# Jiraiya812/Fast-CU-Decision-HEVC

Measured on AMD Instinct MI355X. Metric: CTUs/sec (RDO decision only) at 4K all-intra, higher is better.
Workload: dtype int32+f64

## Files before the change

### fast-cu-decision-hevc_amd/csrc/fcu_engine.h

```cpp
#pragma once
#include <stdint.h>
#include <string.h>
#include <type_traits>
#include "../../include/fcu.h"

#ifdef FCU_EMU
#include <math.h>
#include <stdio.h>
#include <stdlib.h>
#define FCU_DEV static inline
#define FCU_MEMBER inline
#define FCU_NOINLINE
#define FCU_INLINE
#define FCU_TABLE static const
static int g_emu_phase = 0, g_emu_in_phase = 0, g_emu_lane = 0, g_emu_relax = 0;
#define FCU_EMU_RELAX(on) (g_emu_relax = (on))
static inline int fcu_emu_phase_begin() { g_emu_phase++; g_emu_in_phase = 1; g_emu_lane = 0; return 0; }
static inline int fcu_emu_phase_next(int lane) { if (lane + 1 >= 64) g_emu_in_phase = 0; g_emu_lane = lane + 1; return lane + 1; }
template <class T> static inline T fcu_emu_uni(T v, int site, int line)
{
  enum { SITES = 2048, K = 32, B = 16 };
  struct Seen { int phase, first, cur, idx, n; unsigned char vals[K][B]; };
  static Seen seen[SITES];
  if (g_emu_in_phase && !g_emu_relax && sizeof(T) <= B && site < SITES) {
// ... 5 lines not shown
    s.idx++;
  }
  return v;
}
#define FCU_FOR_LANES for (int lane = fcu_emu_phase_begin(); lane < 64; lane = fcu_emu_phase_next(lane))
#define FCU_ATOMIC_ADD(p, v) (*(p) += (v))
#define FCU_ATOMIC_MAX(p, v) do { if (*(p) < (v)) *(p) = (v); } while (0)
#define FCU_ATOMIC_OR(p, v) (*(p) |= (v))
#define FCU_WAVE_ADD(p, v) (*(p) += (v))
#define FCU_WAVE_MIN64(p, v) do { if ((v) < *(p)) *(p) = (v); } while (0)
#define FCU_IN_LDS(p) do { } while (0)
#define FCU_UNI(x) fcu_emu_uni((x), __COUNTER__, __LINE__)
#define FCU_HBM
#define FCU_FLOOR(x) floor(x)
#define FCU_CHECK(c) do { if (!(c)) { fprintf(stderr, "FCU_CHECK failed: %s (line %d)\n", #c, __LINE__); abort(); } } while (0)
#else
#define FCU_DEV __device__ static
#define FCU_MEMBER __device__ inline
#define FCU_NOINLINE __noinline__
#define FCU_INLINE __attribute__((always_inline))
#define FCU_TABLE __device__ static const
#define FCU_FOR_LANES for (int lane = (int)threadIdx.x, fcu_once_ = 1; fcu_once_; fcu_once_ = 0, __syncthreads())
#define FCU_ATOMIC_ADD(p, v) atomicAdd((p), (v))
#define FCU_ATOMIC_MAX(p, v) atomicMax((p), (v))
#define FCU_ATOMIC_OR(p, v) atomicOr((p), (v))
__device__ inline uint32_t fcu_wave_sum(uint32_t v)
{
  v += (uint32_t)__builtin_amdgcn_update_dpp(0, (int)v, 0xb1, 0xf, 0xf, false);
  v += (uint32_t)__builtin_amdgcn_update_dpp(0, (int)v, 0x4e, 0xf, 0xf, false);
  v += (uint32_t)__builtin_amdgcn_update_dpp(0, (int)v, 0x124, 0xf, 0xf, false);
// ... 44 lines not shown
#define FCU_QTIC(v) long long v = clock64()
#define FCU_QTOC(E_, v, idx) do { if (threadIdx.x == 0) (E_).C->prof[idx] += (unsigned long long)(clock64() - v); v = clock64(); } while (0)
#define FCU_TOC(E_, v, idx) do { if ((idx) == 10 && threadIdx.x == 0) (E_).C->prof[idx] += (unsigned long long)(clock64() - v); } while (0)
#define FCU_COUNT(E_, idx, n) do { } while (0)
#elif defined(FCU_PROFILE_INTER)
#define FCU_ITOC(E_, v, idx) do { if (threadIdx.x == 0) (E_).C->prof[idx] += (unsigned long long)(clock64() - v); } while (0)
#define FCU_TOC(E_, v, idx) do { if ((idx) == 10 && threadIdx.x == 0) (E_).C->prof[idx] += (unsigned long long)(clock64() - v); } while (0)
#define FCU_COUNT(E_, idx, n) do { } while (0)
#elif defined(FCU_PROFILE_RDOQ) || defined(FCU_PROFILE_DEPTH)
#define FCU_TOC(E_, v, idx) do { if ((idx) < 11 && threadIdx.x == 0) (E_).C->prof[idx] += (unsigned long long)(clock64() - v); } while (0)
#define FCU_COUNT(E_, idx, n) do { } while (0)
#elif defined(FCU_PROFILE_RMD)
#define FCU_MTOC(E_, v, idx) do { if (threadIdx.x == 0) (E_).C->prof[idx] += (unsigned long long)(clock64() - v); } while (0)
#define FCU_TOC(E_, v, idx) do { if ((idx) < 11 && threadIdx.x == 0) (E_).C->prof[idx] += (unsigned long long)(clock64() - v); } while (0)
#define FCU_COUNT(E_, idx, n) do { } while (0)
#else
#define FCU_TOC(E_, v, idx) do { if (threadIdx.x == 0) (E_).C->prof[idx] += (unsigned long long)(clock64() - v); } while (0)
#define FCU_COUNT(E_, idx, n) do { (E_).C->prof[idx] += (unsigned long long)(n); } while (0)
#endif
#else
#define FCU_TIC(v) do { } while (0)
#define FCU_TOC(E_, v, idx) do { } while (0)
#define FCU_COUNT(E_, idx, n) do { } while (0)
#endif
#ifndef FCU_QTOC
#define FCU_QTIC(v) do { } while (0)
#define FCU_QTOC(E_, v, idx) do { } while (0)
#endif
#ifndef FCU_ITOC
#define FCU_ITOC(E_, v, idx) do { } while (0)
#endif
#ifndef FCU_MTOC
#define FCU_MTOC(E_, v, idx) do { } while (0)
#endif

#include "fcu_tables.h"

struct HotTables { uint32_t bin[256]; uint16_t scan[3][16]; uint8_t scan_cg8[3][4]; uint8_t ctx_ind_map4x4[16]; uint8_t group_idx[32];
                   uint64_t scan4_nib[3], map4_nib; uint32_t cnt_bits[4]; };
#ifdef FCU_EMU
static HotTables g_hot;
#else
__shared__ HotTables g_hot;
#endif

#if defined(FCU_PROFILE_RQT) && !defined(FCU_EMU)
#define FCU_RTIC(v) long long v = clock64()
#define FCU_RTOC(P_, v, idx) do { if (!SER && threadIdx.x == 0) { ((Chain *)((char *)&(P_) - __builtin_offsetof(Chain, p)))->prof[idx] += (unsigned long long)(clock64() - v); v = clock64(); } } while (0)
// ... 101 lines not shown
  Yuv16 resi_cu, resi_best, qt_resi[4];
  Yuv tmp_pred;
  uint8_t me_pred[9][CTU * CTU];
  int16_t me_h[3][72 * 64];
  int par_ps[4];
  int memo_valid[4][MEMO_K], memo_next[4], memo_zero[4][MEMO_K];
  int16_t memo_mv[4][MEMO_K][NPART][2]; int8_t memo_ref[4][MEMO_K][NPART];
  uint8_t memo_tr_idx[4][MEMO_K][NPART], memo_cbf[4][MEMO_K][3][NPART], memo_tskip[4][MEMO_K][3][NPART];
  alignas(16) int16_t memo_coef[MEMO_K * MEMO_POOL], memo_resi[MEMO_K * MEMO_POOL];
};

struct Env { Chain *C; Scratch *G; int cur_ctu, slice_start; };
struct TU { int log2, tr_depth, part, nparts, x, y, off_y, cw, cwo, cx, cy, c_tr_depth, c_code_all, off_c, cu_depth, plast; };

struct Shared {
  Cabac cab[1 + (MAXDEPTH + 1) + MAXLC];
  uint8_t ref5[5][68]; int dc5[5]; uint32_t cm_dist[5];
  union {
    int16_t lane_abs[MAXLC][32];
    RdoqRec rq_rec[16];
    struct {
      int32_t colsum[128];
      union {
        struct { uint8_t ref[264], reff[264]; };
        uint8_t ref5b[5][68];
      };
    };
  };
  union {
    int16_t rq_lv[16];
    uint32_t sad[36];
// ... 21 lines not shown
      uint32_t tz_best; int tz_bx, tz_by, tz_dist, tz_round, tz_point;
      int mrg_buf[5], best_is_skip, me_out[4];
    };
  };
  int pu_best_vc, pu_best_mode, pu_nvc; uint32_t pu_best_dist; double pu_best_cost;
  int t_abs, t_lsp, t_last; uint32_t t_dist;
  int rw_abs, rw_lsp;
  double q_cost[4]; uint32_t q_dist[4];
  int c_best_mode; uint32_t c_best_dist; double c_best_cost; int c_modes[5];
  uint32_t c_dist;
  Env env;
  TU wk_st[4]; int wk_ci[4]; int wk_part[4], wk_child[4];
  double cand_cost[12];
  uint32_t c64_dist[5]; uint8_t c64_cbf[5][4]; int c64_valid;
  uint64_t q_frac[5], t_frac;
  double dec_j0, dec_j1; int dec_cnt, dec_flip;
};

enum { CAB_GOON = 0, CAB_CUR0 = 1, CAB_LANE0 = 1 + (MAXDEPTH + 1) };
enum { EST_CODERS = 7 };
static_assert(EST_CODERS * sizeof(Cabac) >= NCTX_INTRA * 2 * sizeof(uint32_t) && EST_CODERS <= MAXLC, "est table does not fit its lane coders");
#define FCU_EST ((uint32_t *)&g_S.cab[CAB_LANE0 + MAXLC - EST_CODERS])
enum { RMD_STAGE_BYTES = 64 * 8 * 2, RMD_COST_BYTES = 35 * 8 };
static_assert(RMD_STAGE_BYTES + RMD_COST_BYTES <= MAXLC * sizeof(Cabac) && (CAB_LANE0 * sizeof(Cabac)) % 8 == 0, "RMD staging does not fit the lane coders");
#define FCU_RMD_STAGE ((int16_t *)&g_S.cab[CAB_LANE0])
#define FCU_RMD_COST ((double *)((char *)&g_S.cab[CAB_LANE0] + RMD_STAGE_BYTES))
FCU_DEV int ref_key(int px, int py, int log2) { return px | (py << 13) | (log2 << 26); }
#ifdef FCU_EMU
static Shared g_S;
#else
__shared__ Shared g_S;
#endif
FCU_DEV Env env_get() { return FCU_UNI(g_S.env); }
FCU_DEV Cabac *slot_ptr(const Env E, int d, int ci) { return ci == CI_CURR_BEST ? &g_S.cab[CAB_CUR0 + d] : &E.G->slots[d][ci]; }
// ... 1279 lines not shown
  const Env E = env_get(); c = FCU_UNI(c); cu = FCU_UNI(cu); const TU tu = tu_of_key(FCU_UNI(tu_k));
  const int part = tu.part, partSize = cu->part_size[0], log2 = tu.log2;
  cab_reset_bits(c);
  if (part == 0 && E.C->p.slice_type != SLICE_I) { code_skip_flag(E, c, cu, 0); code_pred_mode(c, cu, 0); }
  if (part == 0 && cu->depth[0] == MAXDEPTH) cab_bin(c, partSize == SIZE_2Nx2N, CTX_PARTSIZE);
  if (partSize == SIZE_2Nx2N ? (part == 0) : (tu.tr_depth > 0 && (part & ((cu->nparts >> 2) - 1)) == 0))
    code_luma_dir_bits(c, cu->intra_dir[0][part], g_S.preds);
  if (!(partSize == SIZE_NxN && tu.tr_depth == 0) && log2 != LOG2_MINTU && log2 != min_tu_log2_in_cu(cu->depth[part], cu->part_size[part]))
    cab_bin(c, 0, CTX_SUBDIV + 5 - log2);
  const int cbf = g_S.t_abs > 0;
  cab_bin(c, cbf, CTX_CBF_LUMA + (tu.tr_depth == 0 ? 1 : 0));
  if (cbf) code_coeff_body<1>(c, E.G->p_qscan, 1, g_S.t_lsp, log2, 0, coef_scan_idx(cu->intra_dir[0][part], log2, 0), cu->tskip[0][part], E.C->p, g_S.lane_abs[0]);
  return cab_bits(c);
}

FCU_DEV FCU_NOINLINE void encode_transform(int c, const CuObj *cu, int cuPart, uint32_t root_k)
{
  const Env E = env_get(); c = FCU_UNI(c); cu = FCU_UNI(cu); cuPart = FCU_UNI(cuPart); const TU root = tu_of_key(FCU_UNI(root_k));
  TU *st = g_S.wk_st; int *ci = g_S.wk_ci; int sp = 0;
  st[0] = root; ci[0] = -1;
  while (sp >= 0) {
    const TU tu = st[sp];
    if (ci[sp] < 0) {
      const int part = cuPart + tu.part, trIdx = tu.tr_depth, subdiv = cu->tr_idx[part] > trIdx;
      if (cu->part_size[part] == SIZE_NxN && trIdx == 0) { }
      else if (tu.log2 > LOG2_MAXTU) { }
      else if (tu.log2 == LOG2_MINTU) { }
      else if (tu.log2 == min_tu_log2_in_cu(cu->depth[part], cu->part_size[part])) { }
      else cab_bin(c, subdiv, CTX_SUBDIV + 5 - tu.log2);
      const int first = trIdx == 0;
      for (int comp = 1; comp < 3; comp++)
        if (first || tu.c_code_all)
          if (first || ((cu->cbf[comp][part] >> (trIdx - 1)) & 1)) {
            const int lowest = trIdx + ((subdiv && !(tu.cwo >= 8)) ? 1 : 0);
            cab_bin(c, (cu->cbf[comp][cuPart + tu_part_c(tu)] >> lowest) & 1, CTX_CBF_CHROMA + trIdx);
          }
      if (!subdiv) {
        cab_bin(c, (cu->cbf[0][part] >> trIdx) & 1, CTX_CBF_LUMA + (trIdx == 0 ? 1 : 0));
        for (int comp = 0; comp < 3; comp++) {
          if (comp && tu.cw == 0) continue;
          if (!((cu->cbf[comp][part] >> trIdx) & 1)) continue;
          const int log2 = comp ? ilog2(tu.cw) : tu.log2, pc = cuPart + (comp ? tu_part_c(tu) : tu.part);
          const int dir = comp ? chroma_final_mode(cu, pc) : cu->intra_dir[0][pc];
          const int16_t *coef = cu->coef[comp] + (comp ? (cuPart * 4 + tu.off_c) : (cuPart * 16 + tu.off_y));
          code_coeff_nxn<1>(c, coef, 1, -1, log2, comp, coef_scan_idx(dir, log2, comp), cu->tskip[comp][pc], E.C->p, g_S.lane_abs[0]);
        }
        sp--; continue;
      }
      ci[sp] = 0;
    }
    if (ci[sp] >= 4) { sp--; continue; }
    { TU ch; tu_child(ch, st[sp], ci[sp], 1); ci[sp]++; sp++; st[sp] = ch; ci[sp] = -1; }
  }
}
FCU_DEV void encode_cu_syntax(const Env E, int c, const CuObj *cu, int cuPart, int depth)
{
  if (E.C->p.slice_type != SLICE_I) {
    if (cu->pred_mode[cuPart] == MODE_INTER) { encode_cu_syntax_inter(E, c, cu, cuPart, depth); return; }
    code_skip_flag(E, c, cu, cuPart); code_pred_mode(c, cu, cuPart);
  }
  if (depth == MAXDEPTH) cab_bin(c, cu->part_size[cuPart] == SIZE_2Nx2N, CTX_PARTSIZE);
  code_intra_dir_luma(c, cu, cuPart, 1);
  code_intra_dir_chroma(c, cu->intra_dir[1][cuPart]);
  TU root; tu_root(root, depth);
  encode_transform(c, cu, cuPart, tu_key(root));
}

FCU_DEV FCU_NOINLINE void cu_init(CuObj *cu, int depth, int x, int y, int zidx)
{
  const Env E = env_get(); cu = FCU_UNI(cu); depth = FCU_UNI(depth); x = FCU_UNI(x); y = FCU_UNI(y); zidx = FCU_UNI(zidx);
  const int n = NPART >> (2 * depth), s = CTU >> depth;
  FCU_FOR_LANES {
    if (lane == 0) { cu->cost = FCU_MAX_DOUBLE; cu->dist = 0; cu->bits = 0; cu->bins = 0; cu->depth_cu = depth; cu->x = x; cu->y = y; cu->zidx = zidx; cu->nparts = n; }
    for (int i = lane; i < n; i += 64) {
      cu->depth[i] = (uint8_t)depth; cu->part_size[i] = SIZE_NONE; cu->pred_mode[i] = MODE_NONE; cu->tr_idx[i] = 0;
      cu->tskip[0][i] = cu->tskip[1][i] = cu->tskip[2][i] = 0; cu->cbf[0][i] = cu->cbf[1][i] = cu->cbf[2][i] = 0;
      cu->intra_dir[0][i] = DC; cu->intra_dir[1][i] = 0;
      cu->skip[i] = 0; cu->merge_flag[i] = 0; cu->merge_idx[i] = 0; cu->inter_dir[i] = 0; cu->mvp_idx[i] = -1; cu->ref_idx[i] = -1;
      cu->mv[i][0] = cu->mv[i][1] = 0; cu->mvd[i][0] = cu->mvd[i][1] = 0;
    }
// ... 200 lines not shown
  FCU_FOR_LANES { for (int i = lane; i < N * N; i += 64) { dst[i] = G->ts_coef[comp][i]; const uint8_t v = s[(i / N) * bs + (i % N)]; t[(i / N) * bs + (i % N)] = v; pic[(i / N) * rs + (i % N)] = v; } }
}

template <int LEVEL>
FCU_DEV FCU_NOINLINE void recur_luma_qt(CuObj *cu, uint32_t tu_k, int checkFirst, int reuseVc = -1)
{
  const Env E = env_get(); cu = FCU_UNI(cu); const TU tu = tu_of_key(FCU_UNI(tu_k)); checkFirst = FCU_UNI(checkFirst); reuseVc = FCU_UNI(reuseVc);
  Scratch *G = E.G; const Params &P = E.C->p;
  const int d = FCU_UNI((int)cu->depth_cu), part = tu.part, trDepth = tu.tr_depth, fullDepth = d + trDepth, log2 = tu.log2;
  const int partSize = FCU_UNI((int)cu->part_size[part]);
  const int checkFull = log2 <= LOG2_MAXTU;
  int checkSplit = log2 > min_tu_log2_in_cu(d, partSize);
  if (checkFirst && checkFull) checkSplit = 0;
  int checkTS = P.transform_skip && log2 == 2;
  if (P.ts_fast) checkTS = checkTS && (partSize == SIZE_NxN);
  double singleCost = FCU_MAX_DOUBLE; uint32_t singleDist = 0, singleCbf = 0; int bestModeId = 0; uint64_t singleFrac = 0;

  if (checkFull) {
    if (checkTS) {
      FCU_FOR_LANES cab_copy(slot_ptr(E, fullDepth, CI_QT_TRAFO_ROOT), &g_S.cab[CAB_GOON], lane);
      for (int modeId = 0; modeId < 2; modeId++) {
        FCU_FOR_LANES { for (int i = lane; i < tu.nparts; i += 64) cu->tskip[0][part + i] = (uint8_t)modeId; }
        tu_trial(cu, tu_key(tu), 0, (CAB_GOON), modeId == 0 ? 1 : 2);
        const uint32_t tmpDist = FCU_UNI(g_S.t_dist), tmpCbf = FCU_UNI((uint32_t)((cu->cbf[0][part] >> trDepth) & 1));
        double tmpCost;
        if (modeId == 1 && tmpCbf == 0) tmpCost = FCU_MAX_DOUBLE;
        else {
          { FCU_TIC(t12_); FCU_SERIAL { const uint64_t f0 = g_S.cab[CAB_GOON].frac & 32767; g_S.vc_bits[0] = leaf_luma_bits(CAB_GOON, cu, tu_key(tu)); g_S.t_frac = g_S.cab[CAB_GOON].frac - f0; } FCU_TOC(E, t12_, 12); }
          tmpCost = FCU_UNI(rd_cost(P, g_S.vc_bits[0], tmpDist));
        }
        if (tmpCost < singleCost) {
          singleCost = tmpCost; singleDist = tmpDist; singleCbf = tmpCbf; bestModeId = modeId; singleFrac = FCU_UNI(g_S.t_frac);
          if (bestModeId == 0) { store_intra_result_qt(tu_key(tu), 0); FCU_FOR_LANES cab_copy(slot_ptr(E, fullDepth, CI_TEMP_BEST), &g_S.cab[CAB_GOON], lane); }
        }
        if (modeId == 0) FCU_FOR_LANES cab_copy(&g_S.cab[CAB_GOON], slot_ptr(E, fullDepth, CI_QT_TRAFO_ROOT), lane);
      }
      FCU_FOR_LANES { for (int i = lane; i < tu.nparts; i += 64) cu->tskip[0][part + i] = (uint8_t)bestModeId; }
      if (bestModeId == 0) {
        load_intra_result_qt(cu, tu_key(tu), 0);
        FCU_FOR_LANES { for (int i = lane; i < tu.nparts; i += 64) cu->cbf[0][part + i] = (uint8_t)(singleCbf << trDepth); cab_copy(&g_S.cab[CAB_GOON], slot_ptr(E, fullDepth, CI_TEMP_BEST), lane); }
      }
    } else {
      if (checkSplit) FCU_FOR_LANES cab_copy(slot_ptr(E, fullDepth, CI_QT_TRAFO_ROOT), &g_S.cab[CAB_GOON], lane);
      FCU_FOR_LANES { for (int i = lane; i < tu.nparts; i += 64) cu->tskip[0][part + i] = 0; }
      if (reuseVc >= 0) {
        const int bv = reuseVc, N = 1 << log2, n2 = N * N, layer = LOG2_MAXTU - log2, cbf = FCU_UNI((int)(g_S.vc_abs[bv] > 0));
        FCU_SERIAL { g_S.t_frac = g_S.cab[CAB_LANE0 + g_S.vc_slot[bv]].frac - (g_S.cab[CAB_GOON].frac & 32767); }
        singleFrac = FCU_UNI(g_S.t_frac);
        FCU_FOR_LANES {
          for (int i = lane; i < n2; i += 64) {
            G->qt_coef[0][layer][tu.off_y + i] = (cbf && (i >> 4) <= (g_S.vc_last[bv] >> 4)) ? G->p_qscan[i * g_S.pu_nvc + bv] : (int16_t)0;
            G->qt_rec[layer].y[(tu.y + (i >> log2)) * 64 + tu.x + (i & (N - 1))] = G->p_rec[bv * n2 + i];
          }
          for (int i = lane; i < tu.nparts; i += 64) { cu->tr_idx[part + i] = (uint8_t)trDepth; cu->cbf[0][part + i] = (uint8_t)(cbf << trDepth); }
          cab_copy(&g_S.cab[CAB_GOON], &g_S.cab[CAB_LANE0 + g_S.vc_slot[bv]], lane);
        }
        singleDist = FCU_UNI(g_S.vc_dist[bv]); singleCbf = (uint32_t)cbf; singleCost = FCU_UNI(g_S.vc_cost[bv]);
      } else if (reuseVc <= -2) {
        const int k = -2 - reuseVc, bv = FCU_UNI(g_S.pu_best_vc), N = 1 << log2, n2 = N * N, layer = LOG2_MAXTU - log2, cbf = FCU_UNI((int)g_S.c64_cbf[bv][k]);
        FCU_SERIAL {
          const uint64_t fprev = k ? G->c64_state[bv][k - 1].frac : (slot_ptr(E, d, CI_CURR_BEST)->frac & 32767);
          g_S.t_frac = G->c64_state[bv][k].frac - fprev;
          g_S.vc_bits[0] = (uint32_t)(((fprev & 32767) + g_S.t_frac) >> 15);
          g_S.t_dist = G->c64_distk[bv][k];
        }
        singleFrac = FCU_UNI(g_S.t_frac);
        FCU_FOR_LANES {
          for (int i = lane; i < n2; i += 64) {
            G->qt_coef[0][layer][tu.off_y + i] = G->c64_coef[bv][tu.off_y + i];
            const int o = (tu.y + (i >> log2)) * 64 + tu.x + (i & (N - 1));
            G->qt_rec[layer].y[o] = G->c64_rec[bv][o];
          }
          for (int i = lane; i < tu.nparts; i += 64) { cu->tr_idx[part + i] = (uint8_t)trDepth; cu->cbf[0][part + i] = (uint8_t)(cbf << trDepth); }
          cab_copy(&g_S.cab[CAB_GOON], &G->c64_state[bv][k], lane);
        }
        FCU_SERIAL { g_S.cab[CAB_GOON].frac = (g_S.cab[CAB_GOON].frac & 32767) + ((uint64_t)g_S.vc_bits[0] << 15); }
        singleDist = FCU_UNI(g_S.t_dist); singleCbf = (uint32_t)cbf;
        singleCost = FCU_UNI(rd_cost(P, g_S.vc_bits[0], singleDist));
      } else {
        tu_trial(cu, tu_key(tu), 0, (CAB_GOON), 0);
        singleDist = FCU_UNI(g_S.t_dist);
        if (checkSplit) singleCbf = FCU_UNI((uint32_t)((cu->cbf[0][part] >> trDepth) & 1));
        { FCU_TIC(t12_); FCU_SERIAL { const uint64_t f0 = g_S.cab[CAB_GOON].frac & 32767; g_S.vc_bits[0] = leaf_luma_bits(CAB_GOON, cu, tu_key(tu)); g_S.t_frac = g_S.cab[CAB_GOON].frac - f0; } FCU_TOC(E, t12_, 12); }
        singleFrac = FCU_UNI(g_S.t_frac);
        singleCost = FCU_UNI(rd_cost(P, g_S.vc_bits[0], singleDist));
      }
    }
  }
  if (checkSplit) {
    if constexpr (LEVEL < 3) {
      if (checkFull) { FCU_FOR_LANES { cab_copy(slot_ptr(E, fullDepth, CI_QT_TRAFO_TEST), &g_S.cab[CAB_GOON], lane); } FCU_FOR_LANES { cab_copy(&g_S.cab[CAB_GOON], slot_ptr(E, fullDepth, CI_QT_TRAFO_ROOT), lane); } }
      else FCU_FOR_LANES cab_copy(slot_ptr(E, fullDepth, CI_QT_TRAFO_ROOT), &g_S.cab[CAB_GOON], lane);
      FCU_SERIAL { g_S.q_dist[LEVEL + 1] = 0; g_S.q_cost[LEVEL + 1] = 0; g_S.q_frac[LEVEL + 1] = 0; }
      uint32_t splitCbf = 0;
      int chainOk = LEVEL == 0 && log2 == 6 && !checkFirst && FCU_UNI(g_S.c64_valid);
      for (int i = 0; i < 4; i++) {
        TU c; tu_child(c, tu, i, 0);
        recur_luma_qt<LEVEL + 1>(cu, tu_key(c), checkFirst, chainOk ? -2 - i : -1);
        splitCbf |= FCU_UNI((uint32_t)((cu->cbf[0][c.part] >> c.tr_depth) & 1));
        chainOk = chainOk && FCU_UNI((int)cu->tr_idx[c.part]) == c.tr_depth;
      }
      const uint32_t splitDist = FCU_UNI(g_S.q_dist[LEVEL + 1]);
      const int sumBits = !(partSize == SIZE_NxN && trDepth == 0);
      FCU_FOR_LANES {
        if (splitCbf) for (int o = lane; o < tu.nparts; o += 64) cu->cbf[0][part + o] |= (uint8_t)(1 << trDepth);
        if (!sumBits) cab_copy(&g_S.cab[CAB_GOON], slot_ptr(E, fullDepth, CI_QT_TRAFO_ROOT), lane);
      }
      {
        FCU_TIC(t12_);
        FCU_SERIAL {
          const uint64_t f0 = slot_ptr(E, fullDepth, CI_QT_TRAFO_ROOT)->frac & 32767;
          if (sumBits) {
            g_S.cab[CAB_GOON].frac = f0; g_S.cab[CAB_GOON].bins = 0;
            if (log2 <= LOG2_MAXTU) cab_bin((CAB_GOON), 1, CTX_SUBDIV + 5 - log2);
            g_S.cab[CAB_GOON].frac += g_S.q_frac[LEVEL + 1];
            g_S.vc_bits[0] = (uint32_t)(g_S.cab[CAB_GOON].frac >> 15);
          } else g_S.vc_bits[0] = intra_bits_qt((CAB_GOON), cu, tu_key(tu), 1, 0);
          g_S.t_frac = g_S.cab[CAB_GOON].frac - f0;
        }
        FCU_TOC(E, t12_, 12);
      }
      const double splitCost = FCU_UNI(rd_cost(P, g_S.vc_bits[0], splitDist));
      if (splitCost < singleCost) { FCU_SERIAL { g_S.q_dist[LEVEL] += splitDist; g_S.q_cost[LEVEL] += splitCost; g_S.q_frac[LEVEL] += g_S.t_frac; } return; }
      FCU_FOR_LANES {
        cab_copy(&g_S.cab[CAB_GOON], slot_ptr(E, fullDepth, CI_QT_TRAFO_TEST), lane);
        for (int i = lane; i < tu.nparts; i += 64) { cu->tr_idx[part + i] = (uint8_t)trDepth; cu->cbf[0][part + i] = (uint8_t)(singleCbf << trDepth); cu->tskip[0][part + i] = (uint8_t)bestModeId; }
        const int N = 1 << log2, layer = LOG2_MAXTU - log2;
        const uint8_t *s = G->qt_rec[layer].y + tu.y * 64 + tu.x;
        uint8_t *p = E.C->rec[0] + (cu->y + tu.y) * E.C->stride[0] + cu->x + tu.x; const int rs = E.C->stride[0];
        for (int i = lane; i < N * N; i += 64) p[(i >> log2) * rs + (i & (N - 1))] = s[(i >> log2) * 64 + (i & (N - 1))];
      }
    }
  }
  FCU_SERIAL { g_S.q_dist[LEVEL] += singleDist; g_S.q_cost[LEVEL] += singleCost; g_S.q_frac[LEVEL] += singleFrac; }
}

FCU_DEV FCU_NOINLINE void set_intra_result_luma_qt(CuObj *cu, uint32_t root_k, Yuv *reco)
{
  const Env E = env_get(); cu = FCU_UNI(cu); const TU root = tu_of_key(FCU_UNI(root_k)); reco = FCU_UNI(reco);
  Scratch *G = E.G;
  TU *st = g_S.wk_st; int *ci = g_S.wk_ci; int sp = 0;
  st[0] = root; ci[0] = -1;
  while (sp >= 0) {
    const TU tu = st[sp];
    if (ci[sp] < 0) {
      if (cu->tr_idx[tu.part] == tu.tr_depth) {
        const int N = 1 << tu.log2, layer = LOG2_MAXTU - tu.log2;
        FCU_FOR_LANES {
          for (int i = lane; i < N * N; i += 64) {
// ... 453 lines not shown
      }
    }
  }
}

FCU_DEV int pu_trace_index(int depth, int nxn, int zidx) { return nxn ? 85 + zidx : (depth == 0 ? 0 : depth == 1 ? 1 + (zidx >> 6) : depth == 2 ? 5 + (zidx >> 4) : 21 + (zidx >> 2)); }
FCU_DEV FCU_NOINLINE void est_intra_pred_luma(CuObj *cu)
{
  const Env E = env_get(); cu = FCU_UNI(cu);
  Scratch *G = E.G;
  const int d = cu->depth_cu, partSize = cu->part_size[0];
  const int initTrDepth = partSize == SIZE_2Nx2N ? 0 : 1, numPU = 1 << (2 * initTrDepth), qNumParts = cu->nparts >> 2;
  uint32_t overallDistY = 0;
  TU root; tu_root(root, d);
  Yuv *recoT = &G->reco[d][1 - g_S.reco_best_idx[d]];
  for (int pu = 0; pu < numPU; pu++) {
    TU tu; if (initTrDepth == 0) tu = root; else tu_child(tu, root, pu, 0);
    const int partOffset = tu.part, N = 1 << tu.log2, log2 = tu.log2;
    FCU_SERIAL g_S.c64_valid = 0;
    { FCU_TIC(t_); rmd(cu, tu_key(tu)); FCU_TOC(E, t_, 0); }
    fcu_pu_trace *ptr = FCU_UNI(E.C->pu_trace ? E.C->pu_trace + (size_t)E.cur_ctu * FCU_PUS_PER_CTU + pu_trace_index(d, initTrDepth, cu->zidx + partOffset) : (fcu_pu_trace *)nullptr);
    if (ptr) FCU_SERIAL {
      const int nRmd = k_rd_mode_num[log2 - 2];
      ptr->n_rmd = (uint8_t)nRmd; ptr->n_rd = (uint8_t)g_S.n_rd; ptr->pad = 0;
      for (int i = 0; i < 12; i++) ptr->rd_mode[i] = (uint8_t)(i < g_S.n_rd ? g_S.rd_mode[i] : 0);
      for (int i = 0; i < 8; i++) ptr->rmd_cost[i] = i < nRmd ? g_S.cand_cost[i] : 0.0;
    }
    const int singleTU = log2 <= LOG2_MAXTU;
    if (singleTU) { FCU_TIC(t_); pu_first_pass_batched(cu, tu_key(tu)); FCU_TOC(E, t_, 1); }
    else if (g_S.n_rd <= 5) { FCU_TIC(t_); pu_first_pass_64(cu, tu_key(tu)); FCU_TOC(E, t_, 1); }
    else {
      FCU_SERIAL { g_S.pu_best_cost = FCU_MAX_DOUBLE; g_S.pu_best_mode = 0; g_S.pu_best_dist = 0; }
      const int nc = g_S.n_rd;
      for (int m = 0; m < nc; m++) {
        const int orgMode = g_S.rd_mode[m];
        FCU_FOR_LANES { for (int i = lane; i < tu.nparts; i += 64) cu->intra_dir[0][partOffset + i] = (uint8_t)orgMode; cab_copy(&g_S.cab[CAB_GOON], slot_ptr(E, d, CI_CURR_BEST), lane); if (lane == 0) { g_S.q_dist[0] = 0; g_S.q_cost[0] = 0; } }
        recur_luma_qt<0>(cu, tu_key(tu), 1);
        if (g_S.q_cost[0] < g_S.pu_best_cost) {
          FCU_SERIAL { g_S.pu_best_mode = orgMode; g_S.pu_best_dist = g_S.q_dist[0]; g_S.pu_best_cost = g_S.q_cost[0]; }
          set_intra_result_luma_qt(cu, tu_key(tu), recoT);
          FCU_FOR_LANES { for (int i = lane; i < tu.nparts; i += 64) { G->tmp_tr_idx[i] = cu->tr_idx[partOffset + i]; G->tmp_cbf[i] = cu->cbf[0][partOffset + i]; G->tmp_tskip[i] = cu->tskip[0][partOffset + i]; } }
        }
      }
    }
    if (log2 > min_tu_log2_in_cu(d, partSize)) {
      const int orgMode = g_S.pu_best_mode;
      FCU_FOR_LANES { for (int i = lane; i < tu.nparts; i += 64) cu->intra_dir[0][partOffset + i] = (uint8_t)orgMode; cab_copy(&g_S.cab[CAB_GOON], slot_ptr(E, d, CI_CURR_BEST), lane); if (lane == 0) { g_S.q_dist[0] = 0; g_S.q_cost[0] = 0; } }
      { FCU_TIC(t_); recur_luma_qt<0>(cu, tu_key(tu), 0, singleTU ? g_S.pu_best_vc : -1); FCU_TOC(E, t_, 4); }
      if (g_S.q_cost[0] < g_S.pu_best_cost) {
        FCU_SERIAL { g_S.pu_best_dist = g_S.q_dist[0]; g_S.pu_best_cost = g_S.q_cost[0]; }
        set_intra_result_luma_qt(cu, tu_key(tu), recoT);
        FCU_FOR_LANES { for (int i = lane; i < tu.nparts; i += 64) { G->tmp_tr_idx[i] = cu->tr_idx[partOffset + i]; G->tmp_cbf[i] = cu->cbf[0][partOffset + i]; G->tmp_tskip[i] = cu->tskip[0][partOffset + i]; } }
      }
    }
    overallDistY += g_S.pu_best_dist;
    const int bestMode = g_S.pu_best_mode;
    if (ptr) FCU_SERIAL { ptr->best_mode = (uint8_t)g_S.pu_best_mode; ptr->best_dist = g_S.pu_best_dist; ptr->best_cost = g_S.pu_best_cost; ptr->valid = 1; }
    FCU_FOR_LANES {
      for (int i = lane; i < tu.nparts; i += 64) {
        cu->tr_idx[partOffset + i] = G->tmp_tr_idx[i]; cu->cbf[0][partOffset + i] = G->tmp_cbf[i]; cu->tskip[0][partOffset + i] = G->tmp_tskip[i];
        cu->intra_dir[0][partOffset + i] = (uint8_t)bestMode;
      }
      if (pu != numPU - 1) {
        uint8_t *p = E.C->rec[0] + (cu->y + tu.y) * E.C->stride[0] + cu->x + tu.x; const int rs = E.C->stride[0];
        for (int i = lane; i < N * N; i += 64) p[(i >> log2) * rs + (i & (N - 1))] = recoT->y[(tu.y + (i >> log2)) * 64 + tu.x + (i & (N - 1))];
      }
    }
// ... 312 lines not shown
}
FCU_DEV FCU_NOINLINE void check_rd_cost_intra(int d, int partSize)
{
  const Env E = env_get(); d = FCU_UNI(d); partSize = FCU_UNI(partSize);
  Scratch *G = E.G; const Params &P = E.C->p;
  CuObj *cu = cu_temp(E, d);
  const int n = cu->nparts, s = CTU >> d;
  FCU_FOR_LANES { for (int i = lane; i < n; i += 64) { cu->part_size[i] = (int8_t)partSize; cu->pred_mode[i] = MODE_INTRA; } }
  est_intra_pred_luma(cu);
  {
    const Yuv *recoT = &G->reco[d][1 - g_S.reco_best_idx[d]];
    FCU_FOR_LANES { uint8_t *p = E.C->rec[0] + cu->y * E.C->stride[0] + cu->x; const int rs = E.C->stride[0]; for (int i = lane; i < s * s; i += 64) p[(i / s) * rs + (i % s)] = recoT->y[(i / s) * 64 + (i % s)]; }
  }
  { FCU_TIC(t_); est_intra_pred_chroma(cu); FCU_TOC(E, t_, 6); }
  FCU_TIC(t7_);
  FCU_FOR_LANES {
    if (lane == 0) {
      cab_reset_bits((CAB_GOON));
      encode_cu_syntax(E, (CAB_GOON), cu, 0, d);
      cu->bits = cab_bits((CAB_GOON)); cu->bins = g_S.cab[CAB_GOON].bins;
      cu->cost = rd_cost(P, cu->bits, cu->dist);
    }
  }
  FCU_FOR_LANES cab_copy(slot_ptr(E, d, CI_TEMP_BEST), &g_S.cab[CAB_GOON], lane);
  FCU_TOC(E, t7_, 7);
  check_best_mode(d);
}

FCU_DEV FCU_NOINLINE void check_rd_cost_inter(int d, int partSize, int useMrg)
{
  const Env E = env_get(); d = FCU_UNI(d); partSize = FCU_UNI(partSize); useMrg = FCU_UNI(useMrg);
  CuObj *cu = cu_temp(E, d);
  const int n = cu->nparts;
  FCU_FOR_LANES { for (int i = lane; i < n; i += 64) { cu->part_size[i] = (int8_t)partSize; cu->pred_mode[i] = MODE_INTER; } }
  pred_inter_search(cu, partSize, useMrg);
  { FCU_TIC(p_); encode_res_and_calc_rd_inter_cu(cu, 0); FCU_ITOC(E, p_, 9); }
  check_best_mode(d);
}
FCU_DEV FCU_NOINLINE void check_rd_cost_merge_2nx2n(int d)
{
// ... 367 lines not shown
```

Measured before the change: 19450.

## Reuse luma CABAC state to skip full CU syntax re-encode for 2Nx2N intra

Tracks fractional bits and bin counts through the luma RQT search and keeps the winning luma CABAC context in a new shared coder slot. For 2Nx2N intra CUs, the final CU syntax cost is then built by merging the saved luma contexts with the chroma coder state, so the serial single-lane full encode_cu_syntax pass is skipped. When the CU has more than one transform leaf, only the chroma part is re-encoded, through a new withLuma=0 mode of encode_transform. This adds bookkeeping, one more Cabac in shared memory and a per-byte context merge, and it relies on the merged state matching a full re-encode exactly.

```diff
diff --git a/fast-cu-decision-hevc_amd/csrc/fcu_engine.h b/fast-cu-decision-hevc_amd/csrc/fcu_engine.h
--- a/fast-cu-decision-hevc_amd/csrc/fcu_engine.h
+++ b/fast-cu-decision-hevc_amd/csrc/fcu_engine.h
@@ -43,6 +43,7 @@
 #define FCU_HBM
 #define FCU_FLOOR(x) floor(x)
 #define FCU_CHECK(c) do { if (!(c)) { fprintf(stderr, "FCU_CHECK failed: %s (line %d)\n", #c, __LINE__); abort(); } } while (0)
+static unsigned long long g_emu_cu_paths[3] = { 0, 0, 0 };
 #else
 #define FCU_DEV __device__ static
 #define FCU_MEMBER __device__ inline
@@ -117,6 +118,12 @@
 #define FCU_MTOC(E_, v, idx) do { if (threadIdx.x == 0) (E_).C->prof[idx] += (unsigned long long)(clock64() - v); } while (0)
 #define FCU_TOC(E_, v, idx) do { if ((idx) < 11 && threadIdx.x == 0) (E_).C->prof[idx] += (unsigned long long)(clock64() - v); } while (0)
 #define FCU_COUNT(E_, idx, n) do { } while (0)
+#elif defined(FCU_PROFILE_CUSYN)
+#define FCU_STOC(E_, v, idx) do { if (threadIdx.x == 0) (E_).C->prof[idx] += (unsigned long long)(clock64() - v); } while (0)
+#define FCU_SPATH(E_, path) do { if (threadIdx.x == 0) (E_).C->prof[15] += 1ull << (21 * (path)); } while (0)
+#define FCU_S7_COEFF(E_, v, comp) do { if (g_S.prof_s7 == 1) FCU_STOC(E_, v, (comp) ? 14 : 13); } while (0)
+#define FCU_TOC(E_, v, idx) do { if ((idx) < 11 && threadIdx.x == 0) (E_).C->prof[idx] += (unsigned long long)(clock64() - v); } while (0)
+#define FCU_COUNT(E_, idx, n) do { } while (0)
 #else
 #define FCU_TOC(E_, v, idx) do { if (threadIdx.x == 0) (E_).C->prof[idx] += (unsigned long long)(clock64() - v); } while (0)
 #define FCU_COUNT(E_, idx, n) do { (E_).C->prof[idx] += (unsigned long long)(n); } while (0)
@@ -135,6 +142,11 @@
 #endif
 #ifndef FCU_MTOC
 #define FCU_MTOC(E_, v, idx) do { } while (0)
+#endif
+#ifndef FCU_STOC
+#define FCU_STOC(E_, v, idx) do { } while (0)
+#define FCU_SPATH(E_, path) do { } while (0)
+#define FCU_S7_COEFF(E_, v, comp) do { } while (0)
 #endif
 
 #include "fcu_tables.h"
@@ -266,7 +278,7 @@
 struct TU { int log2, tr_depth, part, nparts, x, y, off_y, cw, cwo, cx, cy, c_tr_depth, c_code_all, off_c, cu_depth, plast; };
 
 struct Shared {
-  Cabac cab[1 + (MAXDEPTH + 1) + MAXLC];
+  Cabac cab[1 + (MAXDEPTH + 1) + MAXLC + 1];
   uint8_t ref5[5][68]; int dc5[5]; uint32_t cm_dist[5];
   union {
     int16_t lane_abs[MAXLC][32];
@@ -318,10 +330,15 @@
   double cand_cost[12];
   uint32_t c64_dist[5]; uint8_t c64_cbf[5][4]; int c64_valid;
   uint64_t q_frac[5], t_frac;
+  uint32_t q_bins[5], t_bins;
+  uint64_t lf_frac; uint32_t lf_bins; int lf_valid;
   double dec_j0, dec_j1; int dec_cnt, dec_flip;
+#ifdef FCU_PROFILE_CUSYN
+  int prof_s7;
+#endif
 };
 
-enum { CAB_GOON = 0, CAB_CUR0 = 1, CAB_LANE0 = 1 + (MAXDEPTH + 1) };
+enum { CAB_GOON = 0, CAB_CUR0 = 1, CAB_LANE0 = 1 + (MAXDEPTH + 1), CAB_LUMA = CAB_LANE0 + MAXLC };
 enum { EST_CODERS = 7 };
 static_assert(EST_CODERS * sizeof(Cabac) >= NCTX_INTRA * 2 * sizeof(uint32_t) && EST_CODERS <= MAXLC, "est table does not fit its lane coders");
 #define FCU_EST ((uint32_t *)&g_S.cab[CAB_LANE0 + MAXLC - EST_CODERS])
@@ -1631,9 +1648,9 @@
   return cab_bits(c);
 }
 
-FCU_DEV FCU_NOINLINE void encode_transform(int c, const CuObj *cu, int cuPart, uint32_t root_k)
-{
-  const Env E = env_get(); c = FCU_UNI(c); cu = FCU_UNI(cu); cuPart = FCU_UNI(cuPart); const TU root = tu_of_key(FCU_UNI(root_k));
+FCU_DEV FCU_NOINLINE void encode_transform(int c, const CuObj *cu, int cuPart, uint32_t root_k, int withLuma)
+{
+  const Env E = env_get(); c = FCU_UNI(c); cu = FCU_UNI(cu); cuPart = FCU_UNI(cuPart); const TU root = tu_of_key(FCU_UNI(root_k)); withLuma = FCU_UNI(withLuma);
   TU *st = g_S.wk_st; int *ci = g_S.wk_ci; int sp = 0;
   st[0] = root; ci[0] = -1;
   while (sp >= 0) {
@@ -1644,7 +1661,7 @@
       else if (tu.log2 > LOG2_MAXTU) { }
       else if (tu.log2 == LOG2_MINTU) { }
       else if (tu.log2 == min_tu_log2_in_cu(cu->depth[part], cu->part_size[part])) { }
-      else cab_bin(c, subdiv, CTX_SUBDIV + 5 - tu.log2);
+      else if (withLuma) cab_bin(c, subdiv, CTX_SUBDIV + 5 - tu.log2);
       const int first = trIdx == 0;
       for (int comp = 1; comp < 3; comp++)
         if (first || tu.c_code_all)
@@ -1653,14 +1670,14 @@
             cab_bin(c, (cu->cbf[comp][cuPart + tu_part_c(tu)] >> lowest) & 1, CTX_CBF_CHROMA + trIdx);
           }
       if (!subdiv) {
-        cab_bin(c, (cu->cbf[0][part] >> trIdx) & 1, CTX_CBF_LUMA + (trIdx == 0 ? 1 : 0));
-        for (int comp = 0; comp < 3; comp++) {
+        if (withLuma) cab_bin(c, (cu->cbf[0][part] >> trIdx) & 1, CTX_CBF_LUMA + (trIdx == 0 ? 1 : 0));
+        for (int comp = withLuma ? 0 : 1; comp < 3; comp++) {
           if (comp && tu.cw == 0) continue;
           if (!((cu->cbf[comp][part] >> trIdx) & 1)) continue;
           const int log2 = comp ? ilog2(tu.cw) : tu.log2, pc = cuPart + (comp ? tu_part_c(tu) : tu.part);
           const int dir = comp ? chroma_final_mode(cu, pc) : cu->intra_dir[0][pc];
           const int16_t *coef = cu->coef[comp] + (comp ? (cuPart * 4 + tu.off_c) : (cuPart * 16 + tu.off_y));
-          code_coeff_nxn<1>(c, coef, 1, -1, log2, comp, coef_scan_idx(dir, log2, comp), cu->tskip[comp][pc], E.C->p, g_S.lane_abs[0]);
+          { FCU_TIC(ts_); code_coeff_nxn<1>(c, coef, 1, -1, log2, comp, coef_scan_idx(dir, log2, comp), cu->tskip[comp][pc], E.C->p, g_S.lane_abs[0]); FCU_S7_COEFF(E, ts_, comp); }
         }
         sp--; continue;
       }
@@ -1680,7 +1697,7 @@
   code_intra_dir_luma(c, cu, cuPart, 1);
   code_intra_dir_chroma(c, cu->intra_dir[1][cuPart]);
   TU root; tu_root(root, depth);
-  encode_transform(c, cu, cuPart, tu_key(root));
+  encode_transform(c, cu, cuPart, tu_key(root), 1);
 }
 
 FCU_DEV FCU_NOINLINE void cu_init(CuObj *cu, int depth, int x, int y, int zidx)
@@ -1911,7 +1928,7 @@
   if (checkFirst && checkFull) checkSplit = 0;
   int checkTS = P.transform_skip && log2 == 2;
   if (P.ts_fast) checkTS = checkTS && (partSize == SIZE_NxN);
-  double singleCost = FCU_MAX_DOUBLE; uint32_t singleDist = 0, singleCbf = 0; int bestModeId = 0; uint64_t singleFrac = 0;
+  double singleCost = FCU_MAX_DOUBLE; uint32_t singleDist = 0, singleCbf = 0, singleBins = 0; int bestModeId = 0; uint64_t singleFrac = 0;
 
   if (checkFull) {
     if (checkTS) {
@@ -1923,11 +1940,11 @@
         double tmpCost;
         if (modeId == 1 && tmpCbf == 0) tmpCost = FCU_MAX_DOUBLE;
         else {
-          { FCU_TIC(t12_); FCU_SERIAL { const uint64_t f0 = g_S.cab[CAB_GOON].frac & 32767; g_S.vc_bits[0] = leaf_luma_bits(CAB_GOON, cu, tu_key(tu)); g_S.t_frac = g_S.cab[CAB_GOON].frac - f0; } FCU_TOC(E, t12_, 12); }
+          { FCU_TIC(t12_); FCU_SERIAL { const uint64_t f0 = g_S.cab[CAB_GOON].frac & 32767; g_S.vc_bits[0] = leaf_luma_bits(CAB_GOON, cu, tu_key(tu)); g_S.t_frac = g_S.cab[CAB_GOON].frac - f0; g_S.t_bins = g_S.cab[CAB_GOON].bins; } FCU_TOC(E, t12_, 12); }
           tmpCost = FCU_UNI(rd_cost(P, g_S.vc_bits[0], tmpDist));
         }
         if (tmpCost < singleCost) {
-          singleCost = tmpCost; singleDist = tmpDist; singleCbf = tmpCbf; bestModeId = modeId; singleFrac = FCU_UNI(g_S.t_frac);
+          singleCost = tmpCost; singleDist = tmpDist; singleCbf = tmpCbf; bestModeId = modeId; singleFrac = FCU_UNI(g_S.t_frac); singleBins = FCU_UNI(g_S.t_bins);
           if (bestModeId == 0) { store_intra_result_qt(tu_key(tu), 0); FCU_FOR_LANES cab_copy(slot_ptr(E, fullDepth, CI_TEMP_BEST), &g_S.cab[CAB_GOON], lane); }
         }
         if (modeId == 0) FCU_FOR_LANES cab_copy(&g_S.cab[CAB_GOON], slot_ptr(E, fullDepth, CI_QT_TRAFO_ROOT), lane);
@@ -1942,8 +1959,8 @@
       FCU_FOR_LANES { for (int i = lane; i < tu.nparts; i += 64) cu->tskip[0][part + i] = 0; }
       if (reuseVc >= 0) {
         const int bv = reuseVc, N = 1 << log2, n2 = N * N, layer = LOG2_MAXTU - log2, cbf = FCU_UNI((int)(g_S.vc_abs[bv] > 0));
-        FCU_SERIAL { g_S.t_frac = g_S.cab[CAB_LANE0 + g_S.vc_slot[bv]].frac - (g_S.cab[CAB_GOON].frac & 32767); }
-        singleFrac = FCU_UNI(g_S.t_frac);
+        FCU_SERIAL { const Cabac *w = &g_S.cab[CAB_LANE0 + g_S.vc_slot[bv]]; g_S.t_frac = w->frac - (g_S.cab[CAB_GOON].frac & 32767); g_S.t_bins = w->bins; }
+        singleFrac = FCU_UNI(g_S.t_frac); singleBins = FCU_UNI(g_S.t_bins);
         FCU_FOR_LANES {
           for (int i = lane; i < n2; i += 64) {
             G->qt_coef[0][layer][tu.off_y + i] = (cbf && (i >> 4) <= (g_S.vc_last[bv] >> 4)) ? G->p_qscan[i * g_S.pu_nvc + bv] : (int16_t)0;
@@ -1958,10 +1975,11 @@
         FCU_SERIAL {
           const uint64_t fprev = k ? G->c64_state[bv][k - 1].frac : (slot_ptr(E, d, CI_CURR_BEST)->frac & 32767);
           g_S.t_frac = G->c64_state[bv][k].frac - fprev;
+          g_S.t_bins = G->c64_state[bv][k].bins - (k ? G->c64_state[bv][k - 1].bins : 0u);
           g_S.vc_bits[0] = (uint32_t)(((fprev & 32767) + g_S.t_frac) >> 15);
           g_S.t_dist = G->c64_distk[bv][k];
         }
-        singleFrac = FCU_UNI(g_S.t_frac);
+        singleFrac = FCU_UNI(g_S.t_frac); singleBins = FCU_UNI(g_S.t_bins);
         FCU_FOR_LANES {
           for (int i = lane; i < n2; i += 64) {
             G->qt_coef[0][layer][tu.off_y + i] = G->c64_coef[bv][tu.off_y + i];
@@ -1978,8 +1996,8 @@
         tu_trial(cu, tu_key(tu), 0, (CAB_GOON), 0);
         singleDist = FCU_UNI(g_S.t_dist);
         if (checkSplit) singleCbf = FCU_UNI((uint32_t)((cu->cbf[0][part] >> trDepth) & 1));
-        { FCU_TIC(t12_); FCU_SERIAL { const uint64_t f0 = g_S.cab[CAB_GOON].frac & 32767; g_S.vc_bits[0] = leaf_luma_bits(CAB_GOON, cu, tu_key(tu)); g_S.t_frac = g_S.cab[CAB_GOON].frac - f0; } FCU_TOC(E, t12_, 12); }
-        singleFrac = FCU_UNI(g_S.t_frac);
+        { FCU_TIC(t12_); FCU_SERIAL { const uint64_t f0 = g_S.cab[CAB_GOON].frac & 32767; g_S.vc_bits[0] = leaf_luma_bits(CAB_GOON, cu, tu_key(tu)); g_S.t_frac = g_S.cab[CAB_GOON].frac - f0; g_S.t_bins = g_S.cab[CAB_GOON].bins; } FCU_TOC(E, t12_, 12); }
+        singleFrac = FCU_UNI(g_S.t_frac); singleBins = FCU_UNI(g_S.t_bins);
         singleCost = FCU_UNI(rd_cost(P, g_S.vc_bits[0], singleDist));
       }
     }
@@ -1988,7 +2006,7 @@
     if constexpr (LEVEL < 3) {
       if (checkFull) { FCU_FOR_LANES { cab_copy(slot_ptr(E, fullDepth, CI_QT_TRAFO_TEST), &g_S.cab[CAB_GOON], lane); } FCU_FOR_LANES { cab_copy(&g_S.cab[CAB_GOON], slot_ptr(E, fullDepth, CI_QT_TRAFO_ROOT), lane); } }
       else FCU_FOR_LANES cab_copy(slot_ptr(E, fullDepth, CI_QT_TRAFO_ROOT), &g_S.cab[CAB_GOON], lane);
-      FCU_SERIAL { g_S.q_dist[LEVEL + 1] = 0; g_S.q_cost[LEVEL + 1] = 0; g_S.q_frac[LEVEL + 1] = 0; }
+      FCU_SERIAL { g_S.q_dist[LEVEL + 1] = 0; g_S.q_cost[LEVEL + 1] = 0; g_S.q_frac[LEVEL + 1] = 0; g_S.q_bins[LEVEL + 1] = 0; }
       uint32_t splitCbf = 0;
       int chainOk = LEVEL == 0 && log2 == 6 && !checkFirst && FCU_UNI(g_S.c64_valid);
       for (int i = 0; i < 4; i++) {
@@ -2010,15 +2028,15 @@
           if (sumBits) {
             g_S.cab[CAB_GOON].frac = f0; g_S.cab[CAB_GOON].bins = 0;
             if (log2 <= LOG2_MAXTU) cab_bin((CAB_GOON), 1, CTX_SUBDIV + 5 - log2);
-            g_S.cab[CAB_GOON].frac += g_S.q_frac[LEVEL + 1];
+            g_S.cab[CAB_GOON].frac += g_S.q_frac[LEVEL + 1]; g_S.cab[CAB_GOON].bins += g_S.q_bins[LEVEL + 1];
             g_S.vc_bits[0] = (uint32_t)(g_S.cab[CAB_GOON].frac >> 15);
           } else g_S.vc_bits[0] = intra_bits_qt((CAB_GOON), cu, tu_key(tu), 1, 0);
-          g_S.t_frac = g_S.cab[CAB_GOON].frac - f0;
+          g_S.t_frac = g_S.cab[CAB_GOON].frac - f0; g_S.t_bins = g_S.cab[CAB_GOON].bins;
         }
         FCU_TOC(E, t12_, 12);
       }
       const double splitCost = FCU_UNI(rd_cost(P, g_S.vc_bits[0], splitDist));
-      if (splitCost < singleCost) { FCU_SERIAL { g_S.q_dist[LEVEL] += splitDist; g_S.q_cost[LEVEL] += splitCost; g_S.q_frac[LEVEL] += g_S.t_frac; } return; }
+      if (splitCost < singleCost) { FCU_SERIAL { g_S.q_dist[LEVEL] += splitDist; g_S.q_cost[LEVEL] += splitCost; g_S.q_frac[LEVEL] += g_S.t_frac; g_S.q_bins[LEVEL] += g_S.t_bins; } return; }
       FCU_FOR_LANES {
         cab_copy(&g_S.cab[CAB_GOON], slot_ptr(E, fullDepth, CI_QT_TRAFO_TEST), lane);
         for (int i = lane; i < tu.nparts; i += 64) { cu->tr_idx[part + i] = (uint8_t)trDepth; cu->cbf[0][part + i] = (uint8_t)(singleCbf << trDepth); cu->tskip[0][part + i] = (uint8_t)bestModeId; }
@@ -2029,7 +2047,7 @@
       }
     }
   }
-  FCU_SERIAL { g_S.q_dist[LEVEL] += singleDist; g_S.q_cost[LEVEL] += singleCost; g_S.q_frac[LEVEL] += singleFrac; }
+  FCU_SERIAL { g_S.q_dist[LEVEL] += singleDist; g_S.q_cost[LEVEL] += singleCost; g_S.q_frac[LEVEL] += singleFrac; g_S.q_bins[LEVEL] += singleBins; }
 }
 
 FCU_DEV FCU_NOINLINE void set_intra_result_luma_qt(CuObj *cu, uint32_t root_k, Yuv *reco)
@@ -2513,10 +2531,11 @@
   uint32_t overallDistY = 0;
   TU root; tu_root(root, d);
   Yuv *recoT = &G->reco[d][1 - g_S.reco_best_idx[d]];
+  const int keepLuma = initTrDepth == 0;
   for (int pu = 0; pu < numPU; pu++) {
     TU tu; if (initTrDepth == 0) tu = root; else tu_child(tu, root, pu, 0);
     const int partOffset = tu.part, N = 1 << tu.log2, log2 = tu.log2;
-    FCU_SERIAL g_S.c64_valid = 0;
+    FCU_SERIAL { g_S.c64_valid = 0; g_S.lf_valid = 0; }
     { FCU_TIC(t_); rmd(cu, tu_key(tu)); FCU_TOC(E, t_, 0); }
     fcu_pu_trace *ptr = FCU_UNI(E.C->pu_trace ? E.C->pu_trace + (size_t)E.cur_ctu * FCU_PUS_PER_CTU + pu_trace_index(d, initTrDepth, cu->zidx + partOffset) : (fcu_pu_trace *)nullptr);
     if (ptr) FCU_SERIAL {
@@ -2533,23 +2552,27 @@
       const int nc = g_S.n_rd;
       for (int m = 0; m < nc; m++) {
         const int orgMode = g_S.rd_mode[m];
-        FCU_FOR_LANES { for (int i = lane; i < tu.nparts; i += 64) cu->intra_dir[0][partOffset + i] = (uint8_t)orgMode; cab_copy(&g_S.cab[CAB_GOON], slot_ptr(E, d, CI_CURR_BEST), lane); if (lane == 0) { g_S.q_dist[0] = 0; g_S.q_cost[0] = 0; } }
+        FCU_FOR_LANES { for (int i = lane; i < tu.nparts; i += 64) cu->intra_dir[0][partOffset + i] = (uint8_t)orgMode; cab_copy(&g_S.cab[CAB_GOON], slot_ptr(E, d, CI_CURR_BEST), lane); if (lane == 0) { g_S.q_dist[0] = 0; g_S.q_cost[0] = 0; g_S.q_frac[0] = 0; g_S.q_bins[0] = 0; } }
         recur_luma_qt<0>(cu, tu_key(tu), 1);
         if (g_S.q_cost[0] < g_S.pu_best_cost) {
-          FCU_SERIAL { g_S.pu_best_mode = orgMode; g_S.pu_best_dist = g_S.q_dist[0]; g_S.pu_best_cost = g_S.q_cost[0]; }
+          FCU_SERIAL { g_S.pu_best_mode = orgMode; g_S.pu_best_dist = g_S.q_dist[0]; g_S.pu_best_cost = g_S.q_cost[0]; g_S.lf_frac = (slot_ptr(E, d, CI_CURR_BEST)->frac & 32767) + g_S.q_frac[0]; g_S.lf_bins = g_S.q_bins[0]; g_S.lf_valid = keepLuma; }
           set_intra_result_luma_qt(cu, tu_key(tu), recoT);
-          FCU_FOR_LANES { for (int i = lane; i < tu.nparts; i += 64) { G->tmp_tr_idx[i] = cu->tr_idx[partOffset + i]; G->tmp_cbf[i] = cu->cbf[0][partOffset + i]; G->tmp_tskip[i] = cu->tskip[0][partOffset + i]; } }
-        }
-      }
+          FCU_FOR_LANES { for (int i = lane; i < tu.nparts; i += 64) { G->tmp_tr_idx[i] = cu->tr_idx[partOffset + i]; G->tmp_cbf[i] = cu->cbf[0][partOffset + i]; G->tmp_tskip[i] = cu->tskip[0][partOffset + i]; } if (keepLuma) cab_copy(&g_S.cab[CAB_LUMA], &g_S.cab[CAB_GOON], lane); }
+        }
+      }
+    }
+    if (keepLuma && (singleTU || g_S.n_rd <= 5)) {
+      const int w = CAB_LANE0 + (singleTU ? FCU_UNI((int)g_S.vc_slot[g_S.pu_best_vc]) : FCU_UNI(g_S.pu_best_vc));
+      FCU_FOR_LANES { cab_copy(&g_S.cab[CAB_LUMA], &g_S.cab[w], lane); if (lane == 0) { g_S.lf_frac = g_S.cab[w].frac; g_S.lf_bins = g_S.cab[w].bins; g_S.lf_valid = 1; } }
     }
     if (log2 > min_tu_log2_in_cu(d, partSize)) {
       const int orgMode = g_S.pu_best_mode;
-      FCU_FOR_LANES { for (int i = lane; i < tu.nparts; i += 64) cu->intra_dir[0][partOffset + i] = (uint8_t)orgMode; cab_copy(&g_S.cab[CAB_GOON], slot_ptr(E, d, CI_CURR_BEST), lane); if (lane == 0) { g_S.q_dist[0] = 0; g_S.q_cost[0] = 0; } }
+      FCU_FOR_LANES { for (int i = lane; i < tu.nparts; i += 64) cu->intra_dir[0][partOffset + i] = (uint8_t)orgMode; cab_copy(&g_S.cab[CAB_GOON], slot_ptr(E, d, CI_CURR_BEST), lane); if (lane == 0) { g_S.q_dist[0] = 0; g_S.q_cost[0] = 0; g_S.q_frac[0] = 0; g_S.q_bins[0] = 0; } }
       { FCU_TIC(t_); recur_luma_qt<0>(cu, tu_key(tu), 0, singleTU ? g_S.pu_best_vc : -1); FCU_TOC(E, t_, 4); }
       if (g_S.q_cost[0] < g_S.pu_best_cost) {
-        FCU_SERIAL { g_S.pu_best_dist = g_S.q_dist[0]; g_S.pu_best_cost = g_S.q_cost[0]; }
+        FCU_SERIAL { g_S.pu_best_dist = g_S.q_dist[0]; g_S.pu_best_cost = g_S.q_cost[0]; g_S.lf_frac = (slot_ptr(E, d, CI_CURR_BEST)->frac & 32767) + g_S.q_frac[0]; g_S.lf_bins = g_S.q_bins[0]; g_S.lf_valid = keepLuma; }
         set_intra_result_luma_qt(cu, tu_key(tu), recoT);
-        FCU_FOR_LANES { for (int i = lane; i < tu.nparts; i += 64) { G->tmp_tr_idx[i] = cu->tr_idx[partOffset + i]; G->tmp_cbf[i] = cu->cbf[0][partOffset + i]; G->tmp_tskip[i] = cu->tskip[0][partOffset + i]; } }
+        FCU_FOR_LANES { for (int i = lane; i < tu.nparts; i += 64) { G->tmp_tr_idx[i] = cu->tr_idx[partOffset + i]; G->tmp_cbf[i] = cu->cbf[0][partOffset + i]; G->tmp_tskip[i] = cu->tskip[0][partOffset + i]; } if (keepLuma) cab_copy(&g_S.cab[CAB_LUMA], &g_S.cab[CAB_GOON], lane); }
       }
     }
     overallDistY += g_S.pu_best_dist;
@@ -2892,16 +2915,81 @@
   }
   { FCU_TIC(t_); est_intra_pred_chroma(cu); FCU_TOC(E, t_, 6); }
   FCU_TIC(t7_);
-  FCU_FOR_LANES {
-    if (lane == 0) {
-      cab_reset_bits((CAB_GOON));
-      encode_cu_syntax(E, (CAB_GOON), cu, 0, d);
-      cu->bits = cab_bits((CAB_GOON)); cu->bins = g_S.cab[CAB_GOON].bins;
-      cu->cost = rd_cost(P, cu->bits, cu->dist);
-    }
-  }
-  FCU_FOR_LANES cab_copy(slot_ptr(E, d, CI_TEMP_BEST), &g_S.cab[CAB_GOON], lane);
+#ifdef FCU_PROFILE_CUSYN
+  if (threadIdx.x == 0) g_S.prof_s7 = partSize == SIZE_2Nx2N ? 1 : 2;
+#endif
+  const int merge = partSize == SIZE_2Nx2N && FCU_UNI(g_S.lf_valid);
+  const int oneLeaf = merge && (FCU_UNI((int)cu->tr_idx[0]) == 0 || d == MAXDEPTH);
+  if (!merge) {
+    FCU_FOR_LANES {
+      if (lane == 0) {
+        cab_reset_bits((CAB_GOON));
+        encode_cu_syntax(E, (CAB_GOON), cu, 0, d);
+        cu->bits = cab_bits((CAB_GOON)); cu->bins = g_S.cab[CAB_GOON].bins;
+        cu->cost = rd_cost(P, cu->bits, cu->dist);
+      }
+    }
+    FCU_FOR_LANES cab_copy(slot_ptr(E, d, CI_TEMP_BEST), &g_S.cab[CAB_GOON], lane);
+    FCU_SPATH(E, 2);
+  } else {
+    if (!oneLeaf) {
+      FCU_FOR_LANES {
+        if (lane == 0) {
+          cab_reset_bits((CAB_GOON));
+          code_intra_dir_chroma((CAB_GOON), cu->intra_dir[1][0]);
+          TU root; tu_root(root, d);
+          encode_transform((CAB_GOON), cu, 0, tu_key(root), 0);
+        }
+      }
+    }
+    const int cc = oneLeaf ? CAB_LANE0 + 5 + FCU_UNI(g_S.c_best_mode) : (int)CAB_GOON;
+    FCU_FOR_LANES {
+      const Cabac *cur = slot_ptr(E, d, CI_CURR_BEST), *lum = &g_S.cab[CAB_LUMA], *chr = &g_S.cab[cc];
+      Cabac *tmp = slot_ptr(E, d, CI_TEMP_BEST), *go = &g_S.cab[CAB_GOON];
+      if (lane < NCTX / 4) {
+        const uint32_t k = ((const uint32_t *)cur->ctx)[lane], l = ((const uint32_t *)lum->ctx)[lane], c = ((const uint32_t *)chr->ctx)[lane];
+        uint32_t m = 0;
+        for (int b = 0; b < 32; b += 8) {
+          const uint32_t kb = (k >> b) & 255, lb = (l >> b) & 255, cb = (c >> b) & 255;
+          FCU_CHECK(lb == kb || cb == kb);
+          m |= (lb != kb ? lb : cb) << b;
+        }
+        ((uint32_t *)tmp->ctx)[lane] = m; ((uint32_t *)go->ctx)[lane] = m;
+      } else if (lane == NCTX / 4) {
+        const uint64_t f = g_S.lf_frac + chr->frac - (cur->frac & 32767);
+        const uint32_t nb = g_S.lf_bins + chr->bins;
+        tmp->frac = f; tmp->bins = nb; tmp->pad_ = 0; go->frac = f; go->bins = nb; go->pad_ = 0;
+        cu->bits = (uint32_t)(f >> 15); cu->bins = nb;
+        cu->cost = rd_cost(P, cu->bits, cu->dist);
+      }
+    }
+    FCU_SPATH(E, oneLeaf ? 0 : 1);
+#ifdef FCU_EMU
+    g_emu_cu_paths[oneLeaf ? 0 : 1]++;
+#ifdef FCU_EMU_CHECK_CU_MERGE
+    FCU_FOR_LANES {
+      if (lane == 0) {
+        const int w = CAB_LANE0 + MAXLC - 1;
+        cab_copy1(&g_S.cab[w], slot_ptr(E, d, CI_CURR_BEST)); cab_reset_bits(w);
+        encode_cu_syntax(E, w, cu, 0, d);
+        const Cabac *tmp = slot_ptr(E, d, CI_TEMP_BEST);
+        FCU_CHECK(memcmp(g_S.cab[w].ctx, tmp->ctx, NCTX) == 0);
+        FCU_CHECK(g_S.cab[w].frac == tmp->frac); FCU_CHECK(g_S.cab[w].bins == tmp->bins);
+        FCU_CHECK(cab_bits(w) == cu->bits); FCU_CHECK(g_S.cab[w].bins == cu->bins);
+        FCU_CHECK(memcmp(&g_S.cab[CAB_GOON], tmp, sizeof(Cabac)) == 0);
+      }
+    }
+#endif
+#endif
+  }
+#ifdef FCU_EMU
+  if (!merge) g_emu_cu_paths[2]++;
+#endif
+#ifdef FCU_PROFILE_CUSYN
+  if (threadIdx.x == 0) g_S.prof_s7 = 0;
+#endif
   FCU_TOC(E, t7_, 7);
+  FCU_STOC(E, t7_, partSize == SIZE_2Nx2N ? 11 : 12);
   check_best_mode(d);
 }
 
```

After: 19970, median of 6. +2.6%, better.
